# JackWoo0831/Yolov7-tracker

Measured on AMD Instinct MI355X. Metric: end-to-end fps (detect+track) YOLOv7-w6@1280 ByteTrack, higher is better.
Workload: dtype f16

## Files before the change

yolov7-tracker_amd/csrc/y7t_conv_patch.hip:

```cpp
#include "y7t_common.h"
#include "y7t_conv_common.h"
#include <stdlib.h>

namespace {

constexpr unsigned kOOB = 0xFF000000u;

template <int TW, int TH, int BN>
struct PatchCfg {
    static constexpr int PIXB = 80;
    static constexpr bool FLAT = (TW == 0);
    static constexpr int PW = TH;
    static constexpr int NPOS = 256 + 2 * PW + 2;
    static constexpr int RP = FLAT ? PW * PIXB : (TW == 16) ? 1536 : (TW + 2) * PIXB;
    static constexpr int PATCH_DMA = FLAT ? (NPOS * PIXB + 1023) / 1024 : ((TH + 2) * RP + 1023) / 1024;
    static constexpr int NPX = (PATCH_DMA + 1) / 2;
    static constexpr int PATCH_BYTES = PATCH_DMA * 1024;
    static constexpr int PPT = (NPX + 6) / 7;
    static constexpr int WROWB = 64;
    static constexpr int W_DMA = BN * WROWB / 1024;
    static constexpr int NWX = W_DMA / 2;
    static constexpr int W_BYTES = W_DMA * 1024;
    static constexpr int NWS = 3;
    static constexpr int W_OFF = 0, P_OFF = NWS * W_BYTES;
    static constexpr int LDS_LOOP = P_OFF + 2 * PATCH_BYTES;
    static constexpr int OROW = BN * 2 + 16;
    static constexpr int LDS_EPI = 256 * OROW;
    static constexpr int BIAS_OFF = LDS_LOOP > LDS_EPI + 1024 ? LDS_LOOP : LDS_EPI + 1024;
    static constexpr int LDS = BIAS_OFF + BN * 4;
    static constexpr int WN = BN / 64, WM = 4 / WN;
    static constexpr int TM = 8 / WM;
    static constexpr int RPT = (TW == 16) ? 2 : 1;
    static constexpr int JOFF = FLAT ? 32 * PIXB : RPT * RP;
};

#define Y7T_PATCH_ISSUE_DMAS() \
            { \
                constexpr bool live = !(ABL & 1); \
                if (wrole) { \
                    const int un = u + 3; \
                    const int ccn = (un / 9), tn = un % 9; \
                    const int cn = c0 + ccn; \
                    if (ABL & 16) issue_w(u % 3, 0, 0, 0, true); \
                    else issue_w(u % 3, ccn == 2 ? cbase + s_pair : cbase + ccn * s_odd, tn / 3, tn % 3, cn < nc32 && live); \
                } else if (t < 7) { \
                _Pragma("unroll") \
                    for (int q = 0; q < C::PPT; ++q) \
                        if (t * C::PPT + q < C::NPX) issue_patch_piece(cc ^ 1, c + 1, t * C::PPT + q, c + 1 < nc32 && live && !(ABL & 32)); \
                } \
            }
template <int TW, int TH, int BN, int ABL>
__global__ void __launch_bounds__(256, 2) k_conv3x3_patch(const Y7TConvArgs p) {
#if defined(__HIP_DEVICE_COMPILE__)
    using C = PatchCfg<TW, TH, BN>;
    static_assert(C::FLAT || TW * TH == 256, "256 output pixels per workgroup");
    constexpr int PIXB = C::PIXB, RP = C::RP, TM = C::TM, RPT = C::RPT;
    constexpr bool FLAT = C::FLAT;
    extern __shared__ __attribute__((aligned(16))) char smem[];
    const int tid = threadIdx.x, lane = tid & 63, wave = __builtin_amdgcn_readfirstlane(tid >> 6);
    const int wn = (C::WN == 2) ? (wave >> 1) : 0, wm = (C::WN == 2) ? (wave & 1) : wave;
    const int l31 = lane & 31, hi32 = lane >> 5;

    int bid = blockIdx.x;
    if (p.xcd_swizzle) {
        const int nwg = gridDim.x, q = nwg >> 3, r = nwg & 7, xcd = bid & 7, idx = bid >> 3;
        bid = (xcd < r ? xcd * (q + 1) : r * (q + 1) + (xcd - r) * q) + idx;
    }
    const int n_tiles_n = p.Cout_pad / BN;
    const int tile_n = bid % n_tiles_n;
    int pt = bid / n_tiles_n;
    int b = 0, h0 = 0, w0 = 0;
    const int g0 = pt * 256;
    const int img_pos = (p.H + 2) * C::PW, strip = p.B * img_pos;
    if (!FLAT) {
        constexpr int TWd = FLAT ? 1 : TW;
        const int tiles_x = (p.W + TWd - 1) / TWd, tiles_y = (p.H + TH - 1) / TH;
        const int txi = pt % tiles_x; pt /= tiles_x;
        const int tyi = pt % tiles_y;
        b = pt / tiles_y; h0 = tyi * TH; w0 = txi * TWd;
    }
    const int n0 = tile_n * BN;

    const __amdgpu_buffer_rsrc_t xr = __builtin_amdgcn_make_buffer_rsrc((void*)p.in, 0, p.in_bytes, 0x00020000);
    const __amdgpu_buffer_rsrc_t wr = __builtin_amdgcn_make_buffer_rsrc((void*)p.w, 0, p.w_bytes, 0x00020000);

    const bool wrole = wave < 2;
    constexpr int NOFF = C::NPX > C::NWX ? C::NPX : C::NWX;
    unsigned off[NOFF];
#pragma unroll
    for (int i = 0; i < NOFF; ++i) {
        unsigned v = kOOB;
        if (wrole) {
            if (i < C::NWX) {
                const int byte = (wave * C::NWX + i) * 1024 + lane * 16;
                const int row = byte >> 6, slot = (byte >> 4) & 3;
                if (p.korder == 2) v = (unsigned)(tile_n * (p.K_pad >> 5) * C::W_BYTES + byte);
                else v = (unsigned)(((n0 + row) * p.K_pad + ((slot ^ ((row >> 2) & 3)) << 3)) * 2);
            }
        } else if (i < C::NPX) {
            int I = (wave - 2) + 2 * i;
            if (I >= C::PATCH_DMA) I = C::PATCH_DMA - 1;
            const int byte = I * 1024 + lane * 16;
            if (FLAT) {
                const int q = byte / PIXB, cs = (byte - q * PIXB) >> 4;
                const int g = g0 - C::PW - 1 + q;
                if (cs < 4 && q < C::NPOS && g >= 0 && g < strip) {
                    const int bb = g / img_pos, rem = g - bb * img_pos;
                    const int yy = rem / C::PW, xx = rem - yy * C::PW;
                    if (yy >= 1 && yy <= p.H && xx >= 1 && xx <= p.W)
                        v = (unsigned)(((((bb * p.H + yy - 1) * p.W + xx - 1) * p.ldin + p.cin_off) + cs * 8) * 2);
                }
            } else {
            const int r = byte / RP, rb = byte - r * RP;
            const int x = rb / PIXB, cs = (rb - x * PIXB) >> 4;
            const int gy = h0 + r - 1, gx = w0 + x - 1;
            const bool ok = r < TH + 2 && x < TW + 2 && cs < 4 && (unsigned)gy < (unsigned)p.H && (unsigned)gx < (unsigned)p.W;
            if (ok) v = (unsigned)(((((b * p.H + gy) * p.W + gx) * p.ldin + p.cin_off) + cs * 8) * 2);
            }
        }
        off[i] = v;
    }

    const int wsw = (l31 >> 2) & 3;
    const char* wlane0 = smem + C::W_OFF + (wn * 64 + l31) * C::WROWB + (((0 + hi32) ^ wsw) << 4);
    const char* wlane1 = smem + C::W_OFF + (wn * 64 + l31) * C::WROWB + (((2 + hi32) ^ wsw) << 4);
    const char* plane = FLAT ? smem + C::P_OFF + (wm * TM * 32 + l31) * PIXB + hi32 * 16
                             : smem + C::P_OFF + (wm * TM * RPT + (TW == 16 ? (l31 >> 4) : 0)) * RP + (TW == 16 ? (l31 & 15) : l31) * PIXB + hi32 * 16;

    const int nc32 = p.Cin >> 5;
    const int s_kh = p.korder == 2 ? 3 * C::W_BYTES : p.korder ? (p.Cin >> 6) * 3 * 128 : 3 * p.Cin * 2;
    const int s_kw = p.korder == 2 ? C::W_BYTES : p.korder ? 128 : p.Cin * 2;
    const int s_odd = p.korder == 2 ? 9 * C::W_BYTES : 64;
    const int s_pair = p.korder == 2 ? 18 * C::W_BYTES : p.korder ? 3 * 128 : 128;
    int cbase = 0;
    auto issue_w = [&](int slot, int coff, int kh, int kw, bool real) {
        const int so = kh * s_kh + kw * s_kw + coff;
#pragma unroll
        for (int i = 0; i < C::NWX; ++i)
            __builtin_amdgcn_raw_ptr_buffer_load_lds(wr, (LDS_AS void*)(smem + C::W_OFF + slot * C::W_BYTES + (wave * C::NWX + i) * 1024), 16,
                                                     real ? off[i] : kOOB, real ? so : 0, 0, 0);
    };
    auto issue_patch_piece = [&](int pb, int c, int i, bool real) {
        const int I = ((wave - 2) + 2 * i < C::PATCH_DMA) ? (wave - 2) + 2 * i : C::PATCH_DMA - 1;
        __builtin_amdgcn_raw_ptr_buffer_load_lds(xr, (LDS_AS void*)(smem + C::P_OFF + pb * C::PATCH_BYTES + I * 1024), 16,
                                                 real ? off[i] : kOOB, c << 6, 0, 0);
    };

    floatx16 acc[2][TM];
#pragma unroll
    for (int i = 0; i < 2; ++i)
#pragma unroll
        for (int j = 0; j < TM; ++j)
#pragma unroll
            for (int e = 0; e < 16; ++e) acc[i][j][e] = 0.f;

    if (tid < BN) ((float*)(smem + C::BIAS_OFF))[tid] = p.bias[n0 + tid];
    if (wrole) {
        issue_w(0, 0, 0, 0, true);
        issue_w(1, 0, 0, 1, true);
        issue_w(2, 0, 0, 2, true);
    } else {
#pragma unroll
        for (int i = 0; i < C::NPX; ++i) issue_patch_piece(0, 0, i, true);
    }

    static_assert(C::PPT * 7 >= C::NPX, "patch pieces fit into taps 0..6");
    static_assert(C::LDS <= 81920, "two workgroups per CU");
    half8 wf[2][2][2], xf[2][2][TM];
    auto read_frags = [&](int buf, int slot, int pb, int kh, int kw) {
        const char* ws0 = wlane0 + slot * C::W_BYTES;
        const char* ws1 = wlane1 + slot * C::W_BYTES;
        const char* ps = plane + pb * C::PATCH_BYTES + kh * RP + kw * PIXB;
        if (ABL & 4) {
#pragma unroll
            for (int ks = 0; ks < 2; ++ks) {
#pragma unroll
                for (int i = 0; i < 2; ++i) asm volatile("" : "=v"(wf[buf][ks][i]));
#pragma unroll
                for (int j = 0; j < TM; ++j) asm volatile("" : "=v"(xf[buf][ks][j]));
            }
            return;
        }
#pragma unroll
        for (int ks = 0; ks < 2; ++ks) {
#pragma unroll
            for (int i = 0; i < 2; ++i) wf[buf][ks][i] = *(const half8*)((ks ? ws1 : ws0) + i * 32 * C::WROWB);
#pragma unroll
            for (int j = 0; j < TM; ++j) xf[buf][ks][j] = *(const half8*)(ps + j * C::JOFF + ks * 32);
        }
    };
    auto mfma_half = [&](int buf, int ks) {
        if (ABL & 2) {
#pragma unroll
            for (int i = 0; i < 2; ++i) asm volatile("" ::"v"(wf[buf][ks][i]));
#pragma unroll
            for (int j = 0; j < TM; ++j) asm volatile("" ::"v"(xf[buf][ks][j]));
            return;
        }
        __builtin_amdgcn_s_setprio(1);
#pragma unroll
        for (int i = 0; i < 2; ++i)
#pragma unroll
            for (int j = 0; j < TM; ++j) acc[i][j] = __builtin_amdgcn_mfma_f32_32x32x16_f16(wf[buf][ks][i], xf[buf][ks][j], acc[i][j], 0, 0, 0);
        __builtin_amdgcn_s_setprio(0);
    };
    if (wrole) asm volatile("s_waitcnt vmcnt(%0)" ::"n"(2 * C::NWX) : "memory");
    else asm volatile("s_waitcnt vmcnt(0)" ::: "memory");
    __builtin_amdgcn_s_barrier();
    read_frags(0, 0, 0, 0, 0);

    for (int c0 = 0; c0 < nc32; c0 += 2) {
#pragma unroll
        for (int u = 0; u < 18; ++u) {
            const int cc = u / 9, t = u % 9;
            const int c = c0 + cc, cur = u & 1;
            if (ABL == 0) {
                const int un = u + 1, tn = un % 9, kh = tn / 3, kw = tn % 3;
                const char* ps = plane + ((un / 9) & 1) * C::PATCH_BYTES + kh * RP + kw * PIXB;
                const char* ws0 = wlane0 + (un % 3) * C::W_BYTES;
                const char* ws1 = wlane1 + (un % 3) * C::W_BYTES;
                __builtin_amdgcn_s_setprio(1);
#pragma unroll
                for (int q = 0; q < 2 * TM; ++q) {
                    const int i = q / TM, j = q % TM;
                    acc[i][j] = __builtin_amdgcn_mfma_f32_32x32x16_f16(wf[cur][0][i], xf[cur][0][j], acc[i][j], 0, 0, 0);
                    if (t < 8) xf[cur ^ 1][q / TM][q % TM] = *(const half8*)(ps + (q % TM) * C::JOFF + (q / TM) * 32);
                    __builtin_amdgcn_sched_barrier(0);
                }
                __builtin_amdgcn_s_setprio(0);
                if (t < 8) asm volatile("s_waitcnt lgkmcnt(%0)" ::"n"(2 * TM) : "memory");
                else asm volatile("s_waitcnt lgkmcnt(0)" ::: "memory");
                if (wrole) asm volatile("s_waitcnt vmcnt(%0)" ::"n"(C::NWX) : "memory");
                else if (t == 8) asm volatile("s_waitcnt vmcnt(0)" ::: "memory");
                __builtin_amdgcn_s_barrier();
                Y7T_PATCH_ISSUE_DMAS()
                __builtin_amdgcn_sched_barrier(0);
                __builtin_amdgcn_s_setprio(1);
#pragma unroll
                for (int q = 0; q < 2 * TM; ++q) {
                    const int i = q / TM, j = q % TM;
                    acc[i][j] = __builtin_amdgcn_mfma_f32_32x32x16_f16(wf[cur][1][i], xf[cur][1][j], acc[i][j], 0, 0, 0);
                    if (q < 4) wf[cur ^ 1][q >> 1][q & 1] = *(const half8*)(((q >> 1) ? ws1 : ws0) + (q & 1) * 32 * C::WROWB);
                    if (t == 8) xf[cur ^ 1][q / TM][q % TM] = *(const half8*)(ps + (q % TM) * C::JOFF + (q / TM) * 32);
                    __builtin_amdgcn_sched_barrier(0);
                }
                __builtin_amdgcn_s_setprio(0);
                continue;
            }
            mfma_half(cur, 0);
            asm volatile("s_waitcnt lgkmcnt(0)" ::: "memory");
            if (wrole) asm volatile("s_waitcnt vmcnt(%0)" ::"n"(C::NWX) : "memory");
            else if (t == 8) asm volatile("s_waitcnt vmcnt(0)" ::: "memory");
            __builtin_amdgcn_s_barrier();
            if (!(ABL & 512)) Y7T_PATCH_ISSUE_DMAS()
            {
                const int un = u + 1, tn = un % 9;
                read_frags(cur ^ 1, un % 3, (un / 9) & 1, tn / 3, tn % 3);
            }
            mfma_half(cur, 1);
            if (ABL & 512) Y7T_PATCH_ISSUE_DMAS()
        }
        cbase += s_pair;
    }

    if (ABL & 8) {
#pragma unroll
        for (int i = 0; i < 2; ++i)
#pragma unroll
            for (int j = 0; j < TM; ++j) asm volatile("" ::"v"(acc[i][j]));
        return;
    }
    constexpr int OROW = C::OROW;
    const float* lbias = (const float*)(smem + C::BIAS_OFF);
    asm volatile("s_waitcnt vmcnt(0)" ::: "memory");
    __syncthreads();
    typedef __attribute__((ext_vector_type(4))) float float4v;
    act_dispatch(p.act, [&](auto act_c) {
    constexpr int ACT = decltype(act_c)::value;
#pragma unroll
    for (int j = 0; j < TM; ++j) {
        const int pix = (wm * TM + j) * 32 + l31;
#pragma unroll
        for (int i = 0; i < 2; ++i) {
            const int nl = wn * 64 + i * 32;
#pragma unroll
            for (int gp = 0; gp < 2; ++gp) {
                unsigned w[2][2];
#pragma unroll
                for (int gg = 0; gg < 2; ++gg) {
                    const int g = gp * 2 + gg;
                    const int n = n0 + nl + 8 * g + 4 * hi32;
                    float v[4];
                    const float4v bv = *(const float4v*)(lbias + (n - n0));
#pragma unroll
                    for (int e = 0; e < 4; ++e) v[e] = act_t<ACT>(acc[i][j][g * 4 + e] + bv[e]);
                    typedef __attribute__((ext_vector_type(2))) _Float16 half2v;
                    half2v h0 = {(half_t)v[0], (half_t)v[1]}, h1 = {(half_t)v[2], (half_t)v[3]};
                    w[gg][0] = __builtin_bit_cast(unsigned, h0);
                    w[gg][1] = __builtin_bit_cast(unsigned, h1);
                }
                auto r0 = __builtin_amdgcn_permlane32_swap(w[0][0], w[1][0], false, false);
                auto r1 = __builtin_amdgcn_permlane32_swap(w[0][1], w[1][1], false, false);
                typedef __attribute__((ext_vector_type(4))) unsigned uint4v;
                uint4v pk = {r0[0], r1[0], r0[1], r1[1]};
                *(uint4v*)(smem + pix * OROW + (nl + 8 * (gp * 2 + hi32)) * 2) = pk;
            }
        }
    }
    });
    int* otab = (int*)(smem + C::LDS_EPI);
    if (FLAT) {
        const int g = g0 + tid;
        int o = -1;
        if (g < strip) {
            const int bb = g / img_pos, rem = g - bb * img_pos;
            const int yy = rem / C::PW, xx = rem - yy * C::PW;
            if (yy >= 1 && yy <= p.H && xx >= 1 && xx <= p.W) o = (bb * p.H + yy - 1) * p.W + xx - 1;
        }
        otab[tid] = o;
    }
    __syncthreads();
    {
        typedef __attribute__((ext_vector_type(4))) unsigned uint4v;
        constexpr int CPP = BN / 8;
        half_t* outp = (half_t*)p.out;
        constexpr int GRP = CPP < 8 ? CPP : 8;
        static_assert(CPP % GRP == 0, "whole groups");
#pragma unroll 1
        for (int c0 = 0; c0 < CPP; c0 += GRP) {
            uint4v v[GRP];
#pragma unroll
            for (int k = 0; k < GRP; ++k) {
                const int cidx = tid + (c0 + k) * 256, pix = cidx / CPP, ch = cidx - pix * CPP;
                v[k] = *(const uint4v*)(smem + pix * OROW + ch * 16);
            }
            __builtin_amdgcn_sched_barrier(0);
#pragma unroll
            for (int k = 0; k < GRP; ++k) {
                const int cidx = tid + (c0 + k) * 256, pix = cidx / CPP, ch = cidx - pix * CPP;
                const int n = n0 + ch * 8;
                long long opix;
                if (FLAT) opix = otab[pix];
                else {
                    constexpr int TWd = FLAT ? 1 : TW;
                    const int r = pix / TWd, x = pix - r * TWd;
                    const int gy = h0 + r, gx = w0 + x;
                    opix = (gy < p.H && gx < p.W) ? (long long)(b * p.H + gy) * p.W + gx : -1;
                }
                if (opix >= 0 && n < p.Cout) *(uint4v*)(outp + (size_t)opix * p.ldout + p.cout_off + n) = v[k];
            }
        }
    }
#endif
}

template <int TW, int TH, int MT>
__global__ void __launch_bounds__(256, 2) k_conv3x3_patch_mt(const Y7TConvArgs p) {
#if defined(__HIP_DEVICE_COMPILE__)
    constexpr int BN = 64;
    using C = PatchCfg<TW, TH, BN>;
    static_assert(!C::FLAT && TW * TH == 256, "256 output pixels per tile");
    constexpr int PIXB = C::PIXB, RP = C::RP, TM = C::TM, RPT = C::RPT;
    constexpr int NWS = 3, WD = 3;
    constexpr int P_OFF = NWS * C::W_BYTES, BIAS_OFF = P_OFF + 2 * C::PATCH_BYTES;
    extern __shared__ __attribute__((aligned(16))) char smem[];
    const int tid = threadIdx.x, lane = tid & 63, wave = __builtin_amdgcn_readfirstlane(tid >> 6);
    const int wm = wave;
    const int l31 = lane & 31, hi32 = lane >> 5;
    int bid = blockIdx.x;
    if (p.xcd_swizzle) {
        const int nwg = gridDim.x, q = nwg >> 3, r = nwg & 7, xcd = bid & 7, idx = bid >> 3;
        bid = (xcd < r ? xcd * (q + 1) : r * (q + 1) + (xcd - r) * q) + idx;
    }
    const int n_tiles_n = p.Cout_pad / BN;
    const int tile_n = bid % n_tiles_n, n0 = tile_n * BN;
    const int tiles_x = (p.W + TW - 1) / TW, tiles_y = (p.H + TH - 1) / TH, ptiles = p.B * tiles_y * tiles_x;
    const int pt_first = (bid / n_tiles_n) * MT;
    const int nt = (ptiles - pt_first) < MT ? (ptiles - pt_first) : MT;

    const __amdgpu_buffer_rsrc_t xr = __builtin_amdgcn_make_buffer_rsrc((void*)p.in, 0, p.in_bytes, 0x00020000);
    const __amdgpu_buffer_rsrc_t wr = __builtin_amdgcn_make_buffer_rsrc((void*)p.w, 0, p.w_bytes, 0x00020000);
    const bool wrole = wave < 2;

    auto patch_off = [&](int pt, unsigned (&o)[C::NPX]) {
        int q = pt;
        const int txi = q % tiles_x; q /= tiles_x;
        const int tyi = q % tiles_y, b = q / tiles_y, h0 = tyi * TH, w0 = txi * TW;
#pragma unroll
        for (int i = 0; i < C::NPX; ++i) {
            int I = (wave - 2) + 2 * i;
            if (I >= C::PATCH_DMA) I = C::PATCH_DMA - 1;
            const int byte = I * 1024 + lane * 16;
            const int r = byte / RP, rb = byte - r * RP;
            const int x = rb / PIXB, cs = (rb - x * PIXB) >> 4;
            const int gy = h0 + r - 1, gx = w0 + x - 1;
            const bool ok = pt < ptiles && r < TH + 2 && x < TW + 2 && cs < 4 && (unsigned)gy < (unsigned)p.H && (unsigned)gx < (unsigned)p.W;
            o[i] = ok ? (unsigned)(((((b * p.H + gy) * p.W + gx) * p.ldin + p.cin_off) + cs * 8) * 2) : kOOB;
        }
    };
    unsigned pc[C::NPX], pn[C::NPX], woff[C::NWX];
#pragma unroll
    for (int i = 0; i < C::NPX; ++i) pc[i] = pn[i] = kOOB;
#pragma unroll
    for (int i = 0; i < C::NWX; ++i) woff[i] = kOOB;
    if (wrole) {
#pragma unroll
        for (int i = 0; i < C::NWX; ++i) {
            const int byte = (wave * C::NWX + i) * 1024 + lane * 16;
            const int row = byte >> 6, slot = (byte >> 4) & 3;
            woff[i] = p.korder == 2 ? (unsigned)(tile_n * (p.K_pad >> 5) * C::W_BYTES + byte)
                                    : (unsigned)(((n0 + row) * p.K_pad + ((slot ^ ((row >> 2) & 3)) << 3)) * 2);
        }
    } else {
        patch_off(pt_first, pc);
        patch_off(pt_first + 1, pn);
    }
    const int wsw = (l31 >> 2) & 3;
    const char* wlane0 = smem + C::W_OFF + l31 * C::WROWB + (((0 + hi32) ^ wsw) << 4);
    const char* wlane1 = smem + C::W_OFF + l31 * C::WROWB + (((2 + hi32) ^ wsw) << 4);
    const char* plane = smem + P_OFF + (wm * TM * RPT + (TW == 16 ? (l31 >> 4) : 0)) * RP + (TW == 16 ? (l31 & 15) : l31) * PIXB + hi32 * 16;

    const int nc32 = p.Cin >> 5, total = nt * nc32;
    const int s_kh = p.korder == 2 ? 3 * C::W_BYTES : p.korder ? (p.Cin >> 6) * 3 * 128 : 3 * p.Cin * 2;
    const int s_kw = p.korder == 2 ? C::W_BYTES : p.korder ? 128 : p.Cin * 2;
    auto chunk_off = [&](int c) -> int {
        return p.korder == 2 ? c * 9 * C::W_BYTES : p.korder ? (c >> 1) * 3 * 128 + (c & 1) * 64 : c * 64;
    };
    auto issue_w = [&](int slot, int c_in_tile, int kh, int kw, bool real) {
        const int so = kh * s_kh + kw * s_kw + chunk_off(c_in_tile);
#pragma unroll
        for (int i = 0; i < C::NWX; ++i)
            __builtin_amdgcn_raw_ptr_buffer_load_lds(wr, (LDS_AS void*)(smem + C::W_OFF + slot * C::W_BYTES + (wave * C::NWX + i) * 1024), 16,
                                                     real ? woff[i] : kOOB, real ? so : 0, 0, 0);
    };
    auto issue_piece = [&](int pb, int i, unsigned voff, int so) {
        const int I = ((wave - 2) + 2 * i < C::PATCH_DMA) ? (wave - 2) + 2 * i : C::PATCH_DMA - 1;
        __builtin_amdgcn_raw_ptr_buffer_load_lds(xr, (LDS_AS void*)(smem + P_OFF + pb * C::PATCH_BYTES + I * 1024), 16, voff, so, 0, 0);
    };

    floatx16 acc[2][TM];
#pragma unroll
    for (int i = 0; i < 2; ++i)
#pragma unroll
        for (int j = 0; j < TM; ++j)
#pragma unroll
            for (int e = 0; e < 16; ++e) acc[i][j][e] = 0.f;
    if (tid < BN) ((float*)(smem + BIAS_OFF))[tid] = p.bias[n0 + tid];
    const float* lbias = (const float*)(smem + BIAS_OFF);
    if (wrole) {
#pragma unroll
        for (int st = 0; st < WD; ++st) issue_w(st, st / 9, (st % 9) / 3, st % 3, st < total * 9);
    } else {
#pragma unroll
        for (int i = 0; i < C::NPX; ++i) issue_piece(0, i, pc[i], 0);
    }
    half8 wf[2][2][2], xf[2][2][TM];
    auto read_frags = [&](int buf, int slot, int pb, int kh, int kw) {
        const char* ws0 = wlane0 + slot * C::W_BYTES;
        const char* ws1 = wlane1 + slot * C::W_BYTES;
        const char* ps = plane + pb * C::PATCH_BYTES + kh * RP + kw * PIXB;
#pragma unroll
        for (int ks = 0; ks < 2; ++ks) {
#pragma unroll
            for (int i = 0; i < 2; ++i) wf[buf][ks][i] = *(const half8*)((ks ? ws1 : ws0) + i * 32 * C::WROWB);
#pragma unroll
            for (int j = 0; j < TM; ++j) xf[buf][ks][j] = *(const half8*)(ps + j * C::JOFF + ks * 32);
        }
    };
    auto mfma_half = [&](int buf, int ks) {
        __builtin_amdgcn_s_setprio(1);
#pragma unroll
        for (int i = 0; i < 2; ++i)
#pragma unroll
            for (int j = 0; j < TM; ++j) acc[i][j] = __builtin_amdgcn_mfma_f32_32x32x16_f16(wf[buf][ks][i], xf[buf][ks][j], acc[i][j], 0, 0, 0);
        __builtin_amdgcn_s_setprio(0);
    };
    if (wrole) asm volatile("s_waitcnt vmcnt(%0)" ::"n"((WD - 1) * C::NWX) : "memory");
    else asm volatile("s_waitcnt vmcnt(0)" ::: "memory");
    __builtin_amdgcn_s_barrier();
    read_frags(0, 0, 0, 0, 0);

    half_t* outp = (half_t*)p.out;
    int ct = 0, tcur = 0;
    for (int c0 = 0; c0 < total; c0 += 2) {
#pragma unroll
        for (int u = 0; u < 18; ++u) {
            const int cc = u / 9, t = u % 9, cur = u & 1;
            mfma_half(cur, 0);
            asm volatile("s_waitcnt lgkmcnt(0)" ::: "memory");
            if (wrole) asm volatile("s_waitcnt vmcnt(%0)" ::"n"((WD - 2) * C::NWX) : "memory");
            else if (t == 8) asm volatile("s_waitcnt vmcnt(0)" ::: "memory");
            __builtin_amdgcn_s_barrier();
            if (wrole) {
                const int un = u + WD, ccn = un / 9, tn = un % 9;
                int cin = ct + ccn;
                if (cin >= nc32) cin -= nc32;
                issue_w(un % NWS, cin, tn / 3, tn % 3, c0 + ccn < total);
            } else if (t < 7) {
                const int cin = ct + cc + 1;
                const bool nxt = cin == nc32;
                const bool live = c0 + cc + 1 < total;
#pragma unroll
                for (int q = 0; q < C::PPT; ++q)
                    if (t * C::PPT + q < C::NPX) {
                        const int i = t * C::PPT + q;
                        issue_piece(cc ^ 1, i, live ? (nxt ? pn[i] : pc[i]) : kOOB, nxt ? 0 : cin << 6);
                    }
            }
            {
                const int un = u + 1, tn = un % 9;
                read_frags(cur ^ 1, un % NWS, (un / 9) & 1, tn / 3, tn % 3);
            }
            mfma_half(cur, 1);
        }
        ct += 2;
        if (ct == nc32) {
            int q = pt_first + tcur;
            const int txi = q % tiles_x; q /= tiles_x;
            const int tyi = q % tiles_y, b = q / tiles_y, h0 = tyi * TH, w0 = txi * TW;
            act_dispatch(p.act, [&](auto act_c) {
            constexpr int ACT = decltype(act_c)::value;
            typedef __attribute__((ext_vector_type(4))) float float4v;
#pragma unroll
            for (int j = 0; j < TM; ++j) {
                const int pix = (wm * TM + j) * 32 + l31;
                const int r = pix / TW, x = pix - r * TW;
                const int gy = h0 + r, gx = w0 + x;
                const bool okp = gy < p.H && gx < p.W;
                half_t* orow = outp + ((size_t)(b * p.H + gy) * p.W + gx) * p.ldout + p.cout_off + n0;
#pragma unroll
                for (int i = 0; i < 2; ++i) {
#pragma unroll
                    for (int gp = 0; gp < 2; ++gp) {
                        unsigned w[2][2];
#pragma unroll
                        for (int gg = 0; gg < 2; ++gg) {
                            const int g = gp * 2 + gg;
                            const int nl = i * 32 + 8 * g + 4 * hi32;
                            float v[4];
                            const float4v bv = *(const float4v*)(lbias + nl);
#pragma unroll
                            for (int e = 0; e < 4; ++e) v[e] = act_t<ACT>(acc[i][j][g * 4 + e] + bv[e]);
                            typedef __attribute__((ext_vector_type(2))) _Float16 half2v;
                            half2v h0v = {(half_t)v[0], (half_t)v[1]}, h1v = {(half_t)v[2], (half_t)v[3]};
                            w[gg][0] = __builtin_bit_cast(unsigned, h0v);
                            w[gg][1] = __builtin_bit_cast(unsigned, h1v);
                        }
                        auto r0 = __builtin_amdgcn_permlane32_swap(w[0][0], w[1][0], false, false);
                        auto r1 = __builtin_amdgcn_permlane32_swap(w[0][1], w[1][1], false, false);
                        typedef __attribute__((ext_vector_type(4))) unsigned uint4v;
                        const uint4v pk = {r0[0], r1[0], r0[1], r1[1]};
                        const int nn = i * 32 + 8 * (gp * 2 + hi32);
                        if (okp && n0 + nn < p.Cout) *(uint4v*)(orow + nn) = pk;
                    }
#pragma unroll
                    for (int e = 0; e < 16; ++e) acc[i][j][e] = 0.f;
                }
            }
            });
            ct = 0;
            ++tcur;
            if (!wrole) {
#pragma unroll
                for (int i = 0; i < C::NPX; ++i) pc[i] = pn[i];
                patch_off(pt_first + tcur + 1, pn);
            }
        }
    }
#endif
}

template <int TW, int TH, int MT>
int launch_patch_mt(const Y7TConvArgs& a, hipStream_t s) {
    using C0 = PatchCfg<TW, TH, 64>;
    constexpr int lds = 3 * C0::W_BYTES + 2 * C0::PATCH_BYTES + 64 * 4;
    static_assert(lds <= 81920, "two workgroups per CU");
    static Y7TOncePerDevice attr;
    if (int e_ = y7t_once_per_device(attr, [&]() -> int {
        Y7T_HIP_CHECK(hipFuncSetAttribute((const void*)k_conv3x3_patch_mt<TW, TH, MT>, hipFuncAttributeMaxDynamicSharedMemorySize, lds));
        return 0;
    })) return e_;
    const int ptiles = a.B * ((a.H + TH - 1) / TH) * ((a.W + TW - 1) / TW);
    hipLaunchKernelGGL((k_conv3x3_patch_mt<TW, TH, MT>), dim3(((ptiles + MT - 1) / MT) * (a.Cout_pad / 64)), dim3(256), lds, s, a);
    Y7T_LAUNCH_CHECK();
    y7t_note_kernel("patch_mt<%d,%d,%d>", TW, TH, MT);
    return 0;
}

template <int TW, int TH, int BN, int ABL = 0>
int launch_patch(const Y7TConvArgs& a, hipStream_t s) {
    using C = PatchCfg<TW, TH, BN>;
    static Y7TOncePerDevice attr;
    if (int e_ = y7t_once_per_device(attr, [&]() -> int {
        Y7T_HIP_CHECK(hipFuncSetAttribute((const void*)k_conv3x3_patch<TW, TH, BN, ABL>, hipFuncAttributeMaxDynamicSharedMemorySize, C::LDS));
        return 0;
    })) return e_;
    const int ptiles = C::FLAT ? (a.B * (a.H + 2) * C::PW + 255) / 256 : a.B * ((a.H + TH - 1) / TH) * ((a.W + (C::FLAT ? 1 : TW) - 1) / (C::FLAT ? 1 : TW));
    const int tiles = ptiles * (a.Cout_pad / BN);
    hipLaunchKernelGGL((k_conv3x3_patch<TW, TH, BN, ABL>), dim3(tiles), dim3(256), C::LDS, s, a);
    Y7T_LAUNCH_CHECK();
    if (C::FLAT) y7t_note_kernel("patch_strip<%d,%d>%s", C::PW, BN, ABL == 2048 ? " burst-reads" : "");
    else y7t_note_kernel("patch<%d,%d,%d>%s", TW, TH, BN, ABL == 2048 ? " burst-reads" : "");
    return 0;
}

}

int y7t_conv_patch_try(const Y7TConvArgs& a, hipStream_t s) {
    static int mode = -1;
    if (mode < 0) mode = y7t_exp_switch("Y7T_CONV_PATCH", 1);
    const bool eligible = a.KH == 3 && a.KW == 3 && a.stride == 1 && a.pad == 1 && a.Cin % 64 == 0 && !a.out_f32 && !(a.Cout & 7) && !(a.ldout & 7) &&
                          !(a.cout_off & 7) && a.Ho == a.H && a.Wo == a.W && a.in_bytes <= kOOB - (1u << 24) && a.w_bytes <= kOOB - (1u << 24);
    if (a.korder == 2 && (!eligible || !mode)) {
        y7t_set_error("conv: weights are in panel order (korder 2) but the layer cannot run on the patch kernel");
        return Y7T_E_ARG;
    }
    if (!mode || !eligible) return 0;
    auto eff = [&](int tw, int th) {
        const int tx = (a.W + tw - 1) / tw, ty = (a.H + th - 1) / th;
        return (double)(a.W * a.H) / ((double)tx * tw * ty * th);
    };
    const double e16 = eff(16, 16), e32 = eff(32, 8);
    const bool use16 = e16 >= e32;
    const bool wide = a.Cout_pad % 128 == 0 && !a.panel64;
    const double eflat = (a.W == 40 || a.W == 20) ? (double)(a.W * a.H) / ((a.W + 2) * (a.H + 2)) : 0.0;
    if (!a.force_patch && a.korder != 2 && (long long)a.B * a.H * a.W * (a.Cout_pad / (wide ? 128 : 64)) < 256ll * 256) return 0;
    const int abl = Y7T_ABLATE ? a.ablate : 0;
    if (eflat > (use16 ? e16 : e32) && eflat >= 0.8 && (!abl || abl == 2048)) {
        int rcf;
#if Y7T_ABLATE
        if (abl == 2048) {
            if (a.W == 40) rcf = wide ? launch_patch<0, 42, 128, 2048>(a, s) : launch_patch<0, 42, 64, 2048>(a, s);
            else rcf = wide ? launch_patch<0, 22, 128, 2048>(a, s) : launch_patch<0, 22, 64, 2048>(a, s);
        } else
#endif
        if (a.W == 40) rcf = wide ? launch_patch<0, 42, 128>(a, s) : launch_patch<0, 42, 64>(a, s);
        else rcf = wide ? launch_patch<0, 22, 128>(a, s) : launch_patch<0, 22, 64>(a, s);
        return rcf ? rcf : 1;
    }
    if (!a.force_patch && a.korder != 2 && (use16 ? e16 : e32) < 0.8) return 0;
    int rc;
#if Y7T_ABLATE
    if (abl == 2048) {
        if (use16) rc = wide ? launch_patch<16, 16, 128, 2048>(a, s) : launch_patch<16, 16, 64, 2048>(a, s);
        else rc = wide ? launch_patch<32, 8, 128, 2048>(a, s) : launch_patch<32, 8, 64, 2048>(a, s);
        return rc ? rc : 1;
    }
    if (abl && use16 && wide) {
        switch (abl) {
        case 1: return launch_patch<16, 16, 128, 1>(a, s) ? -1 : 1;
        case 2: return launch_patch<16, 16, 128, 2>(a, s) ? -1 : 1;
        case 4: return launch_patch<16, 16, 128, 4>(a, s) ? -1 : 1;
        case 8: return launch_patch<16, 16, 128, 8>(a, s) ? -1 : 1;
        case 15: return launch_patch<16, 16, 128, 15>(a, s) ? -1 : 1;
        case 16: return launch_patch<16, 16, 128, 16>(a, s) ? -1 : 1;
        case 32: return launch_patch<16, 16, 128, 32>(a, s) ? -1 : 1;
        case 48: return launch_patch<16, 16, 128, 48>(a, s) ? -1 : 1;
        default: break;
        }
    }
#endif
    static int mt = -1;
    if (mt < 0) mt = y7t_exp_switch("Y7T_CONV_PATCH_MT", 1);
    const int ptiles = a.B * ((a.H + (use16 ? 15 : 7)) / (use16 ? 16 : 8)) * ((a.W + (use16 ? 15 : 31)) / (use16 ? 16 : 32));
    if (!wide && mt && !abl && (ptiles * (a.Cout_pad / 64) >= 4 * 2048 || a.force_patch)) {
        rc = use16 ? launch_patch_mt<16, 16, 4>(a, s) : launch_patch_mt<32, 8, 4>(a, s);
        return rc ? rc : 1;
    }
    if (use16) rc = wide ? launch_patch<16, 16, 128>(a, s) : launch_patch<16, 16, 64>(a, s);
    else rc = wide ? launch_patch<32, 8, 128>(a, s) : launch_patch<32, 8, 64>(a, s);
    return rc ? rc : 1;
}
```

Measured before the change: 2435.

## Add persistent work-stealing form of the 3x3 patch conv kernel

Adds a persistent variant of the 3x3 patch convolution kernel. It launches two workgroups per CU, and each pulls tiles from a global atomic counter. The next tile's patch, weight and bias loads are issued during the last K-chunk of the current tile, and the epilogue writes straight from registers. The aim is to remove per-tile launch and prologue cost and tail imbalance across many small workgroups. It also bypasses the multi-tile kernel whenever the persistent path is eligible. In exchange it adds atomic traffic, a counter reset protocol and a more complex prefetch control flow.

```diff
diff --git a/yolov7-tracker_amd/csrc/y7t_conv_patch.hip b/yolov7-tracker_amd/csrc/y7t_conv_patch.hip
--- a/yolov7-tracker_amd/csrc/y7t_conv_patch.hip
+++ b/yolov7-tracker_amd/csrc/y7t_conv_patch.hip
@@ -28,6 +28,7 @@
     static constexpr int LDS_EPI = 256 * OROW;
     static constexpr int BIAS_OFF = LDS_LOOP > LDS_EPI + 1024 ? LDS_LOOP : LDS_EPI + 1024;
     static constexpr int LDS = BIAS_OFF + BN * 4;
+    static constexpr int BIAS2_OFF = LDS, TKT_OFF = BIAS2_OFF + BN * 4, LDS_P = TKT_OFF + 16;
     static constexpr int WN = BN / 64, WM = 4 / WN;
     static constexpr int TM = 8 / WM;
     static constexpr int RPT = (TW == 16) ? 2 : 1;
@@ -42,18 +43,25 @@
                     const int ccn = (un / 9), tn = un % 9; \
                     const int cn = c0 + ccn; \
                     if (ABL & 16) issue_w(u % 3, 0, 0, 0, true); \
-                    else issue_w(u % 3, ccn == 2 ? cbase + s_pair : cbase + ccn * s_odd, tn / 3, tn % 3, cn < nc32 && live); \
+                    else if (PERS && ccn == 2 && cn >= nc32) issue_w(u % 3, wso_n, tn / 3, tn % 3, has_next);    \
+                    else issue_w(u % 3, (ccn == 2 ? cbase + s_pair : cbase + ccn * s_odd) + wso, tn / 3, tn % 3, cn < nc32 && live); \
                 } else if (t < 7) { \
                 _Pragma("unroll") \
                     for (int q = 0; q < C::PPT; ++q) \
-                        if (t * C::PPT + q < C::NPX) issue_patch_piece(cc ^ 1, c + 1, t * C::PPT + q, c + 1 < nc32 && live && !(ABL & 32)); \
+                        if (t * C::PPT + q < C::NPX) { \
+                            if (PERS && cc == 1 && c + 1 >= nc32) {    \
+                                if (has_next) off[t * C::PPT + q] = patch_src(t * C::PPT + q, g0_n, b_n, h0_n, w0_n); \
+                                issue_patch_piece(0, 0, t * C::PPT + q, has_next); \
+                            } else issue_patch_piece(cc ^ 1, c + 1, t * C::PPT + q, c + 1 < nc32 && live && !(ABL & 32)); \
+                        } \
                 } \
             }
-template <int TW, int TH, int BN, int ABL>
+template <int TW, int TH, int BN, int ABL, bool PERS = false>
 __global__ void __launch_bounds__(256, 2) k_conv3x3_patch(const Y7TConvArgs p) {
 #if defined(__HIP_DEVICE_COMPILE__)
     using C = PatchCfg<TW, TH, BN>;
     static_assert(C::FLAT || TW * TH == 256, "256 output pixels per workgroup");
+    static_assert(!PERS || ABL == 0, "the persistent form has no ablation instances");
     constexpr int PIXB = C::PIXB, RP = C::RP, TM = C::TM, RPT = C::RPT;
     constexpr bool FLAT = C::FLAT;
     extern __shared__ __attribute__((aligned(16))) char smem[];
@@ -67,19 +75,22 @@
         bid = (xcd < r ? xcd * (q + 1) : r * (q + 1) + (xcd - r) * q) + idx;
     }
     const int n_tiles_n = p.Cout_pad / BN;
-    const int tile_n = bid % n_tiles_n;
+    int tile_n = bid % n_tiles_n;
     int pt = bid / n_tiles_n;
     int b = 0, h0 = 0, w0 = 0;
-    const int g0 = pt * 256;
+    int g0 = pt * 256;
     const int img_pos = (p.H + 2) * C::PW, strip = p.B * img_pos;
+    constexpr int TWd = FLAT ? 1 : TW;
+    const int tiles_x = (p.W + TWd - 1) / TWd, tiles_y = (p.H + TH - 1) / TH;
     if (!FLAT) {
-        constexpr int TWd = FLAT ? 1 : TW;
-        const int tiles_x = (p.W + TWd - 1) / TWd, tiles_y = (p.H + TH - 1) / TH;
         const int txi = pt % tiles_x; pt /= tiles_x;
         const int tyi = pt % tiles_y;
         b = pt / tiles_y; h0 = tyi * TH; w0 = txi * TWd;
     }
-    const int n0 = tile_n * BN;
+    int n0 = tile_n * BN;
+    const int n_tiles = (FLAT ? (strip + 255) / 256 : p.B * tiles_y * tiles_x) * n_tiles_n;
+    int g0_n = 0, b_n = 0, h0_n = 0, w0_n = 0, n0_n = 0, wso = 0, wso_n = 0, it = 0;
+    bool has_next = false;
 
     const __amdgpu_buffer_rsrc_t xr = __builtin_amdgcn_make_buffer_rsrc((void*)p.in, 0, p.in_bytes, 0x00020000);
     const __amdgpu_buffer_rsrc_t wr = __builtin_amdgcn_make_buffer_rsrc((void*)p.w, 0, p.w_bytes, 0x00020000);
@@ -87,6 +98,33 @@
     const bool wrole = wave < 2;
     constexpr int NOFF = C::NPX > C::NWX ? C::NPX : C::NWX;
     unsigned off[NOFF];
+    auto patch_src = [&](int i, int g0_, int b_, int h0_, int w0_) -> unsigned {
+        unsigned v = kOOB;
+        int I = (wave - 2) + 2 * i;
+        if (I >= C::PATCH_DMA) I = C::PATCH_DMA - 1;
+        int ln = lane;
+        if (PERS) asm volatile("" : "+v"(ln));
+        const int byte = I * 1024 + ln * 16;
+        if (FLAT) {
+            const int q = byte / PIXB, cs = (byte - q * PIXB) >> 4;
+            const int g = g0_ - C::PW - 1 + q;
+            if (cs < 4 && q < C::NPOS && g >= 0 && g < strip) {
+                const int bb = g / img_pos, rem = g - bb * img_pos;
+                const int yy = rem / C::PW, xx = rem - yy * C::PW;
+                if (yy >= 1 && yy <= p.H && xx >= 1 && xx <= p.W)
+                    v = (unsigned)(((((bb * p.H + yy - 1) * p.W + xx - 1) * p.ldin + p.cin_off) + cs * 8) * 2);
+            }
+        } else {
+            const int r = byte / RP, rb = byte - r * RP;
+            const int x = rb / PIXB, cs = (rb - x * PIXB) >> 4;
+            const int gy = h0_ + r - 1, gx = w0_ + x - 1;
+            const bool ok = r < TH + 2 && x < TW + 2 && cs < 4 && (unsigned)gy < (unsigned)p.H && (unsigned)gx < (unsigned)p.W;
+            if (ok) v = (unsigned)(((((b_ * p.H + gy) * p.W + gx) * p.ldin + p.cin_off) + cs * 8) * 2);
+        }
+        return v;
+    };
+    auto w_tile_so = [&](int tn_) -> int { return p.korder == 2 ? tn_ * (p.K_pad >> 5) * C::W_BYTES : tn_ * BN * p.K_pad * 2; };
+    if (PERS) wso = w_tile_so(tile_n);
 #pragma unroll
     for (int i = 0; i < NOFF; ++i) {
         unsigned v = kOOB;
@@ -94,30 +132,10 @@
             if (i < C::NWX) {
                 const int byte = (wave * C::NWX + i) * 1024 + lane * 16;
                 const int row = byte >> 6, slot = (byte >> 4) & 3;
-                if (p.korder == 2) v = (unsigned)(tile_n * (p.K_pad >> 5) * C::W_BYTES + byte);
-                else v = (unsigned)(((n0 + row) * p.K_pad + ((slot ^ ((row >> 2) & 3)) << 3)) * 2);
-            }
-        } else if (i < C::NPX) {
-            int I = (wave - 2) + 2 * i;
-            if (I >= C::PATCH_DMA) I = C::PATCH_DMA - 1;
-            const int byte = I * 1024 + lane * 16;
-            if (FLAT) {
-                const int q = byte / PIXB, cs = (byte - q * PIXB) >> 4;
-                const int g = g0 - C::PW - 1 + q;
-                if (cs < 4 && q < C::NPOS && g >= 0 && g < strip) {
-                    const int bb = g / img_pos, rem = g - bb * img_pos;
-                    const int yy = rem / C::PW, xx = rem - yy * C::PW;
-                    if (yy >= 1 && yy <= p.H && xx >= 1 && xx <= p.W)
-                        v = (unsigned)(((((bb * p.H + yy - 1) * p.W + xx - 1) * p.ldin + p.cin_off) + cs * 8) * 2);
-                }
-            } else {
-            const int r = byte / RP, rb = byte - r * RP;
-            const int x = rb / PIXB, cs = (rb - x * PIXB) >> 4;
-            const int gy = h0 + r - 1, gx = w0 + x - 1;
-            const bool ok = r < TH + 2 && x < TW + 2 && cs < 4 && (unsigned)gy < (unsigned)p.H && (unsigned)gx < (unsigned)p.W;
-            if (ok) v = (unsigned)(((((b * p.H + gy) * p.W + gx) * p.ldin + p.cin_off) + cs * 8) * 2);
-            }
-        }
+                if (p.korder == 2) v = (unsigned)((PERS ? 0 : tile_n * (p.K_pad >> 5) * C::W_BYTES) + byte);
+                else v = (unsigned)((((PERS ? 0 : n0) + row) * p.K_pad + ((slot ^ ((row >> 2) & 3)) << 3)) * 2);
+            }
+        } else if (i < C::NPX) v = patch_src(i, g0, b, h0, w0);
         off[i] = v;
     }
 
@@ -156,13 +174,17 @@
 
     if (tid < BN) ((float*)(smem + C::BIAS_OFF))[tid] = p.bias[n0 + tid];
     if (wrole) {
-        issue_w(0, 0, 0, 0, true);
-        issue_w(1, 0, 0, 1, true);
-        issue_w(2, 0, 0, 2, true);
+        issue_w(0, wso, 0, 0, true);
+        issue_w(1, wso, 0, 1, true);
+        issue_w(2, wso, 0, 2, true);
     } else {
 #pragma unroll
         for (int i = 0; i < C::NPX; ++i) issue_patch_piece(0, 0, i, true);
     }
+    volatile int* const tkt = (volatile int*)(smem + C::TKT_OFF);
+    const __amdgpu_buffer_rsrc_t br = __builtin_amdgcn_make_buffer_rsrc((void*)p.bias, 0, (unsigned)p.Cout_pad * 4u, 0x00020000);
+    int fetched = 0;
+    if (PERS && tid == 128) fetched = atomicAdd(p.tile_ctr, 1);
 
     static_assert(C::PPT * 7 >= C::NPX, "patch pieces fit into taps 0..6");
     static_assert(C::LDS <= 81920, "two workgroups per CU");
@@ -206,9 +228,30 @@
     };
     if (wrole) asm volatile("s_waitcnt vmcnt(%0)" ::"n"(2 * C::NWX) : "memory");
     else asm volatile("s_waitcnt vmcnt(0)" ::: "memory");
+    if (PERS && tid == 128) tkt[0] = fetched;
+    if (PERS && wave == 2) asm volatile("s_waitcnt lgkmcnt(0)" ::: "memory");
     __builtin_amdgcn_s_barrier();
     read_frags(0, 0, 0, 0, 0);
 
+    for (;;) {
+    if (PERS) {
+        const int tile_next = (int)gridDim.x + __builtin_amdgcn_readfirstlane(tkt[it & 1]);
+        has_next = tile_next < n_tiles;
+        if (has_next) {
+            const int tn_ = tile_next % n_tiles_n;
+            int q = tile_next / n_tiles_n;
+            g0_n = q * 256;
+            if (!FLAT) {
+                const int txi = q % tiles_x; q /= tiles_x;
+                const int tyi = q % tiles_y;
+                b_n = q / tiles_y; h0_n = tyi * TH; w0_n = txi * TWd;
+            }
+            n0_n = tn_ * BN;
+            wso_n = w_tile_so(tn_);
+            if (tid == 128) fetched = atomicAdd(p.tile_ctr, 1);
+        }
+        cbase = 0;
+    }
     for (int c0 = 0; c0 < nc32; c0 += 2) {
 #pragma unroll
         for (int u = 0; u < 18; ++u) {
@@ -232,8 +275,16 @@
                 else asm volatile("s_waitcnt lgkmcnt(0)" ::: "memory");
                 if (wrole) asm volatile("s_waitcnt vmcnt(%0)" ::"n"(C::NWX) : "memory");
                 else if (t == 8) asm volatile("s_waitcnt vmcnt(0)" ::: "memory");
+                if (PERS && u == 8) {
+                    if (tid == 128 && c0 == 0 && has_next) tkt[(it + 1) & 1] = fetched;
+                }
                 __builtin_amdgcn_s_barrier();
                 Y7T_PATCH_ISSUE_DMAS()
+                if (PERS && u == 0) {
+                    if (c0 == 0 && has_next && !wrole && wave - 2 < BN / 64)
+                        __builtin_amdgcn_raw_ptr_buffer_load_lds(br, (LDS_AS void*)(smem + ((it & 1) ? C::BIAS_OFF : C::BIAS2_OFF) + (wave - 2) * 256), 4,
+                                                                 (unsigned)((n0_n + (wave - 2) * 64 + lane) * 4), 0, 0, 0);
+                }
                 __builtin_amdgcn_sched_barrier(0);
                 __builtin_amdgcn_s_setprio(1);
 #pragma unroll
@@ -261,6 +312,72 @@
             if (ABL & 512) Y7T_PATCH_ISSUE_DMAS()
         }
         cbase += s_pair;
+    }
+    if (!PERS) break;
+    {
+        const float* lb = (const float*)(smem + ((it & 1) ? C::BIAS2_OFF : C::BIAS_OFF));
+        half_t* outp = (half_t*)p.out;
+        act_dispatch(p.act, [&](auto act_c) {
+        constexpr int ACT = decltype(act_c)::value;
+        typedef __attribute__((ext_vector_type(4))) float float4v;
+        typedef __attribute__((ext_vector_type(4))) unsigned uint4v;
+#pragma unroll
+        for (int j = 0; j < TM; ++j) {
+            const int pix = (wm * TM + j) * 32 + l31;
+            long long opix = -1;
+            if (FLAT) {
+                const int g = g0 + pix;
+                if (g < strip) {
+                    const int bb = g / img_pos, rem = g - bb * img_pos;
+                    const int yy = rem / C::PW, xx = rem - yy * C::PW;
+                    if (yy >= 1 && yy <= p.H && xx >= 1 && xx <= p.W) opix = (long long)(bb * p.H + yy - 1) * p.W + xx - 1;
+                }
+            } else {
+                const int r = pix / TWd, x = pix - r * TWd;
+                const int gy = h0 + r, gx = w0 + x;
+                if (gy < p.H && gx < p.W) opix = (long long)(b * p.H + gy) * p.W + gx;
+            }
+            half_t* orow = outp + (size_t)(opix < 0 ? 0 : opix) * p.ldout + p.cout_off + n0;
+#pragma unroll
+            for (int i = 0; i < 2; ++i) {
+                const int nl = wn * 64 + i * 32;
+#pragma unroll
+                for (int gp = 0; gp < 2; ++gp) {
+                    unsigned w[2][2];
+#pragma unroll
+                    for (int gg = 0; gg < 2; ++gg) {
+                        const int g = gp * 2 + gg;
+                        float v[4];
+                        const float4v bv = *(const float4v*)(lb + nl + 8 * g + 4 * hi32);
+#pragma unroll
+                        for (int e = 0; e < 4; ++e) v[e] = act_t<ACT>(acc[i][j][g * 4 + e] + bv[e]);
+                        typedef __attribute__((ext_vector_type(2))) _Float16 half2v;
+                        half2v h0v = {(half_t)v[0], (half_t)v[1]}, h1v = {(half_t)v[2], (half_t)v[3]};
+                        w[gg][0] = __builtin_bit_cast(unsigned, h0v);
+                        w[gg][1] = __builtin_bit_cast(unsigned, h1v);
+                    }
+                    auto r0 = __builtin_amdgcn_permlane32_swap(w[0][0], w[1][0], false, false);
+                    auto r1 = __builtin_amdgcn_permlane32_swap(w[0][1], w[1][1], false, false);
+                    const uint4v pk = {r0[0], r1[0], r0[1], r1[1]};
+                    const int nn = nl + 8 * (gp * 2 + hi32);
+                    if (opix >= 0 && n0 + nn < p.Cout) *(uint4v*)(orow + nn) = pk;
+                    __builtin_amdgcn_sched_barrier(0);
+                }
+#pragma unroll
+                for (int e = 0; e < 16; ++e) acc[i][j][e] = 0.f;
+            }
+        }
+        });
+    }
+    if (!has_next) break;
+    tile_n = n0_n / BN; n0 = n0_n; wso = wso_n;
+    g0 = g0_n; b = b_n; h0 = h0_n; w0 = w0_n;
+    ++it;
+    }
+    if (PERS) {
+        asm volatile("s_waitcnt vmcnt(0)" ::: "memory");
+        if (tid == 128 && atomicAdd(p.tile_ctr + Y7T_TILE_CTR_DONE, 1) == (int)gridDim.x - 1) { p.tile_ctr[0] = 0; p.tile_ctr[Y7T_TILE_CTR_DONE] = 0; }
+        return;
     }
 
     if (ABL & 8) {
@@ -597,6 +714,23 @@
     })) return e_;
     const int ptiles = C::FLAT ? (a.B * (a.H + 2) * C::PW + 255) / 256 : a.B * ((a.H + TH - 1) / TH) * ((a.W + (C::FLAT ? 1 : TW) - 1) / (C::FLAT ? 1 : TW));
     const int tiles = ptiles * (a.Cout_pad / BN);
+    if constexpr (ABL == 0) {
+        static const int dyn_env = y7t_switch("Y7T_CONV_WS_DYN", 1);
+        const int slots = 2 * y7t_num_cus();
+        if (a.tile_ctr && dyn_env && tiles >= 2 * slots && a.w_bytes <= (1u << 24)) {
+            static_assert(C::LDS_P <= 81920, "two workgroups per CU");
+            static Y7TOncePerDevice attrp;
+            if (int e_ = y7t_once_per_device(attrp, [&]() -> int {
+                Y7T_HIP_CHECK(hipFuncSetAttribute((const void*)k_conv3x3_patch<TW, TH, BN, 0, true>, hipFuncAttributeMaxDynamicSharedMemorySize, C::LDS_P));
+                return 0;
+            })) return e_;
+            hipLaunchKernelGGL((k_conv3x3_patch<TW, TH, BN, 0, true>), dim3(slots), dim3(256), C::LDS_P, s, a);
+            Y7T_LAUNCH_CHECK();
+            if (C::FLAT) y7t_note_kernel("patch_strip<%d,%d> dyn", C::PW, BN);
+            else y7t_note_kernel("patch<%d,%d,%d> dyn", TW, TH, BN);
+            return 0;
+        }
+    }
     hipLaunchKernelGGL((k_conv3x3_patch<TW, TH, BN, ABL>), dim3(tiles), dim3(256), C::LDS, s, a);
     Y7T_LAUNCH_CHECK();
     if (C::FLAT) y7t_note_kernel("patch_strip<%d,%d>%s", C::PW, BN, ABL == 2048 ? " burst-reads" : "");
@@ -663,7 +797,9 @@
     static int mt = -1;
     if (mt < 0) mt = y7t_exp_switch("Y7T_CONV_PATCH_MT", 1);
     const int ptiles = a.B * ((a.H + (use16 ? 15 : 7)) / (use16 ? 16 : 8)) * ((a.W + (use16 ? 15 : 31)) / (use16 ? 16 : 32));
-    if (!wide && mt && !abl && (ptiles * (a.Cout_pad / 64) >= 4 * 2048 || a.force_patch)) {
+    static const int dyn_env = y7t_switch("Y7T_CONV_WS_DYN", 1);
+    const bool pers = a.tile_ctr && dyn_env && ptiles * (a.Cout_pad / 64) >= 4 * y7t_num_cus() && a.w_bytes <= (1u << 24);
+    if (!wide && mt && !abl && !pers && (ptiles * (a.Cout_pad / 64) >= 4 * 2048 || a.force_patch)) {
         rc = use16 ? launch_patch_mt<16, 16, 4>(a, s) : launch_patch_mt<32, 8, 4>(a, s);
         return rc ? rc : 1;
     }
```

Result: slower. 2404 (-1.2%).
